# atomicarchitects/equiformer

Hardware: AMD Instinct MI355X
Metric: molecules/sec (train step) QM9 L_max=2, 6 blocks (higher is better)
Workload: dtype f32; 1 GPU; QM9 graph_attention_transformer_nonlinear_l2 train step (radius graph + fwd + L1 + bwd + AdamW), 128 molecules/GPU x 18 atoms, r=5.0, num_basis=128, alpha_drop=0.2; global_batch=128, nodes_per_gpu=2304, edges_per_gpu=25354, parallelism=dp1, matrix_mode=split, hip_graph=True, hip_graph_replays=452, hip_graph_eager_steps=3

## Files before the change

equiformer_amd/csrc/edge.hip:

```cpp
#include "common.h"
#include "prof.h"

namespace {

__global__ __launch_bounds__(256) void gather_add_kernel(const float* __restrict__ a, const float* __restrict__ b,
                                                         const int* __restrict__ src, const int* __restrict__ dst,
                                                         float* __restrict__ msg, long total4, int D4) {
  const long idx = (long)blockIdx.x * blockDim.x + threadIdx.x;
  if (idx >= total4) return;
  const long e = idx / D4;
  const int c = (int)(idx - e * D4);
  float4 v = reinterpret_cast<const float4*>(a)[(long)src[e] * D4 + c];
  if (b) {
    const float4 w = reinterpret_cast<const float4*>(b)[(long)dst[e] * D4 + c];
    v.x += w.x, v.y += w.y, v.z += w.z, v.w += w.w;
  }
  reinterpret_cast<float4*>(msg)[idx] = v;
}

__global__ __launch_bounds__(128) void segment_sum_kernel(const float* __restrict__ x, const int* __restrict__ ptr,
                                                          const int* __restrict__ perm, float* __restrict__ out, int D,
                                                          float scale, int accumulate) {
  const int n = blockIdx.x;
  const int beg = ptr[n], end = ptr[n + 1];
// ... 392 lines not shown
}

__global__ void attn_bwd_half_kernel(const float* __restrict__ alpha, const float* __restrict__ value,
                                     const int* __restrict__ row_ptr, const float* __restrict__ d_out,
                                     float* __restrict__ d_value, float* __restrict__ d_logit, const HeadTab T,
                                     float drop_p, unsigned long long seed0,
    const unsigned long long* __restrict__ seed_off) {
  const unsigned long long seed = seed0 + (seed_off ? *seed_off : 0ull);
  const int n = blockIdx.x;
  const int h = threadIdx.x >> 6, lane = threadIdx.x & 63;
  const int half = lane >> 5, gl = lane & 31;
  const int beg = row_ptr[n], end = row_ptr[n + 1];
  const int H = T.H, D4 = T.D >> 2;
  const int col4 = (gl < T.G) ? head_col(T, h, gl) >> 2 : -1;
  const float4 z4 = make_float4(0.f, 0.f, 0.f, 0.f);
  const float4 go = (col4 >= 0) ? reinterpret_cast<const float4*>(d_out)[(long)n * D4 + col4] : z4;
  float s_acc = 0.f;
  for (int e0 = beg; e0 < end; e0 += 4) {
    const int ea = e0 + half, eb = e0 + 2 + half;
    const bool va = ea < end, vb = eb < end;
    const float aa = va ? alpha[(long)ea * H + h] : 0.f, ab = vb ? alpha[(long)eb * H + h] : 0.f;
    const float4 xa = (va && col4 >= 0) ? reinterpret_cast<const float4*>(value)[(long)ea * D4 + col4] : z4;
    const float4 xb = (vb && col4 >= 0) ? reinterpret_cast<const float4*>(value)[(long)eb * D4 + col4] : z4;
    const float keepa = keep_scale(seed, (unsigned long long)ea * H + h, drop_p);
    const float keepb = keep_scale(seed, (unsigned long long)eb * H + h, drop_p);
    float pa = xa.x * go.x + xa.y * go.y + xa.z * go.z + xa.w * go.w;
    float pb = xb.x * go.x + xb.y * go.y + xb.z * go.z + xb.w * go.w;
    if (va && col4 >= 0) {
      const float k = aa * keepa;
      reinterpret_cast<float4*>(d_value)[(long)ea * D4 + col4] = make_float4(k * go.x, k * go.y, k * go.z, k * go.w);
    }
    if (vb && col4 >= 0) {
      const float k = ab * keepb;
      reinterpret_cast<float4*>(d_value)[(long)eb * D4 + col4] = make_float4(k * go.x, k * go.y, k * go.z, k * go.w);
    }
#pragma unroll
    for (int o = 16; o > 0; o >>= 1) pa += __shfl_xor(pa, o), pb += __shfl_xor(pb, o);
    const float da = pa * keepa, db = pb * keepb;
    float contrib = aa * da + ab * db;
    contrib += __shfl_xor(contrib, 32);
    s_acc += contrib;
    if (gl == 0) {
      if (va) d_logit[(long)ea * H + h] = da;
      if (vb) d_logit[(long)eb * H + h] = db;
    }
  }
  __threadfence_block();
  for (int e = beg + lane; e < end; e += 64) {
    const float da = d_logit[(long)e * H + h];
    d_logit[(long)e * H + h] = alpha[(long)e * H + h] * (da - s_acc);
  }
}

__global__ void attn_bwd_kernel(const float* __restrict__ alpha, const float* __restrict__ value,
                                const int* __restrict__ row_ptr, const float* __restrict__ d_out,
                                float* __restrict__ d_value, float* __restrict__ d_logit, const HeadTab T, float drop_p,
                                unsigned long long seed0,
    const unsigned long long* __restrict__ seed_off) {
  const unsigned long long seed = seed0 + (seed_off ? *seed_off : 0ull);
  const int n = blockIdx.x;
  const int h = threadIdx.x >> 6, lane = threadIdx.x & 63;
  const int beg = row_ptr[n], end = row_ptr[n + 1];
  const int H = T.H, D4 = T.D >> 2;
  int col4[MAX_SLOTS];
  float4 go[MAX_SLOTS];
#pragma unroll
  for (int s = 0; s < MAX_SLOTS; ++s) {
    const int g = lane + 64 * s;
    col4[s] = (g < T.G) ? head_col(T, h, g) >> 2 : -1;
    go[s] = (col4[s] >= 0) ? reinterpret_cast<const float4*>(d_out)[(long)n * D4 + col4[s]]
                           : make_float4(0.f, 0.f, 0.f, 0.f);
  }
  float s_acc = 0.f;
  for (int e = beg; e < end; ++e) {
    const float a = alpha[(long)e * H + h];
    const float keep = keep_scale(seed, (unsigned long long)e * H + h, drop_p);
    const float ak = a * keep;
    float part = 0.f;
#pragma unroll
    for (int s = 0; s < MAX_SLOTS; ++s)
      if (col4[s] >= 0) {
        const float4 v = reinterpret_cast<const float4*>(value)[(long)e * D4 + col4[s]];
        part += v.x * go[s].x + v.y * go[s].y + v.z * go[s].z + v.w * go[s].w;
        float4 dv;
        dv.x = ak * go[s].x, dv.y = ak * go[s].y, dv.z = ak * go[s].z, dv.w = ak * go[s].w;
        reinterpret_cast<float4*>(d_value)[(long)e * D4 + col4[s]] = dv;
      }
    const float da = wave_sum(part) * keep;
    s_acc = fmaf(a, da, s_acc);
    if (lane == 0) d_logit[(long)e * H + h] = da;
  }
  __threadfence_block();
  for (int e = beg + lane; e < end; e += 64) {
    const float da = d_logit[(long)e * H + h];
    d_logit[(long)e * H + h] = alpha[(long)e * H + h] * (da - s_acc);
  }
}

HeadTab make_headtab(const eqf_irreps& ir, int H, int* err) {
  HeadTab T{};
  *err = 0;
  T.nseg = ir.nseg;
  T.H = H;
  int off = 0, g = 0;
  for (int s = 0; s < ir.nseg; ++s) {
    T.off[s] = off;
// ... 156 lines not shown
  if (N <= 0) return 0;
  const int pid = eqf_prof_begin("attn_fwd", (hipStream_t)stream, 0.0, 0.0);
  if (T.G <= 32)
    hipLaunchKernelGGL(attn_fwd_half_kernel, dim3(N), dim3(64 * H), 0, (hipStream_t)stream, logit, value, row_ptr, alpha,
                       out, T, drop_p, seed, seed_off);
  else
    hipLaunchKernelGGL(attn_fwd_kernel, dim3(N), dim3(64 * H), 0, (hipStream_t)stream, logit, value, row_ptr, alpha, out,
                       T, drop_p, seed, seed_off);
  eqf_prof_end(pid, (hipStream_t)stream);
  EQF_CHECK_LAUNCH();
  return 0;
}

int eqf_attn_aggregate_fwd(const float* logit, const float* value, const int* row_ptr, float* alpha, float* out, int N,
                           int H, const eqf_irreps* irreps, float drop_p, unsigned long long seed, void* stream) {
  return attn_aggregate_fwd_impl(logit, value, row_ptr, alpha, out, N, H, irreps, drop_p, seed, nullptr, stream);
}
int eqf_attn_aggregate_fwd_dseed(const float* logit, const float* value, const int* row_ptr, float* alpha, float* out, int N,
                                 int H, const eqf_irreps* irreps, float drop_p, unsigned long long seed,
                                 const unsigned long long* seed_offset, void* stream) {
  return attn_aggregate_fwd_impl(logit, value, row_ptr, alpha, out, N, H, irreps, drop_p, seed, seed_offset, stream);
}

static int attn_aggregate_bwd_impl(const float* alpha, const float* value, const int* row_ptr, const float* d_out,
                                   float* d_value, float* d_logit, int N, int H, const eqf_irreps* irreps, float drop_p,
                                   unsigned long long seed, const unsigned long long* seed_off, void* stream) {
  if (!alpha || !value || !row_ptr || !d_out || !d_value || !d_logit || !irreps || H < 1) return EQF_E_BADARG;
  int err;
  const HeadTab T = make_headtab(*irreps, H, &err);
  if (err) return err;
  if (N <= 0) return 0;
  const int pid = eqf_prof_begin("attn_bwd", (hipStream_t)stream, 0.0, 0.0);
  if (T.G <= 32)
    hipLaunchKernelGGL(attn_bwd_half_kernel, dim3(N), dim3(64 * H), 0, (hipStream_t)stream, alpha, value, row_ptr, d_out,
                       d_value, d_logit, T, drop_p, seed, seed_off);
  else
    hipLaunchKernelGGL(attn_bwd_kernel, dim3(N), dim3(64 * H), 0, (hipStream_t)stream, alpha, value, row_ptr, d_out,
                       d_value, d_logit, T, drop_p, seed, seed_off);
  eqf_prof_end(pid, (hipStream_t)stream);
  EQF_CHECK_LAUNCH();
  return 0;
}
int eqf_attn_aggregate_bwd(const float* alpha, const float* value, const int* row_ptr, const float* d_out,
                           float* d_value, float* d_logit, int N, int H, const eqf_irreps* irreps, float drop_p,
                           unsigned long long seed, void* stream) {
  return attn_aggregate_bwd_impl(alpha, value, row_ptr, d_out, d_value, d_logit, N, H, irreps, drop_p, seed, nullptr, stream);
}
int eqf_attn_aggregate_bwd_dseed(const float* alpha, const float* value, const int* row_ptr, const float* d_out,
                                 float* d_value, float* d_logit, int N, int H, const eqf_irreps* irreps, float drop_p,
                                 unsigned long long seed, const unsigned long long* seed_offset, void* stream) {
  return attn_aggregate_bwd_impl(alpha, value, row_ptr, d_out, d_value, d_logit, N, H, irreps, drop_p, seed, seed_offset, stream);
}

}
```

equiformer_amd/lib.py:

```python
import ctypes
import os

_HERE = os.path.dirname(os.path.abspath(__file__))
LIB_PATH = os.path.join(_HERE, "libequiformer_hip.so")
if os.environ.get("EQF_LIB_VARIANT"):
    LIB_PATH = os.path.join(_HERE, "libequiformer_hip_%s.so" % os.environ["EQF_LIB_VARIANT"])

EQF_MAX_SEG = 8
EQF_MAX_PATHS = 72

c_fp = ctypes.c_void_p
c_int = ctypes.c_int


class EqfIrreps(ctypes.Structure):
    _fields_ = [("nseg", c_int), ("l", c_int * EQF_MAX_SEG), ("mul", c_int * EQF_MAX_SEG), ("odd", c_int * EQF_MAX_SEG)]


class EqfRows(ctypes.Structure):
    _fields_ = [("d", c_int), ("ld", c_int), ("inner", c_int)]


class EqfGemmDesc(ctypes.Structure):
    _fields_ = [("A", c_fp), ("B", c_fp), ("C", c_fp), ("bias", c_fp), ("ra", EqfRows), ("rc", EqfRows),
# ... 52 lines not shown
    "eqf_dtp_coupling_bwd": [c_fp, c_fp, _P_PATHS, c_fp, c_int, c_fp],
    "eqf_dtp_linear_fwd": [c_fp, c_fp, c_fp, _P_PATHS, _PP, c_fp, c_fp, _P_IRR, c_int, c_fp],
    "eqf_dtp_linear_wgrad": [c_fp, c_fp, c_fp, _P_PATHS, c_fp, _P_IRR, _PP, c_int, c_fp],
    "eqf_sfc_fwd": [c_fp, c_fp, c_fp, _P_PATHS, _PP, c_fp, c_fp, c_fp, c_fp, _P_IRR, c_fp, c_int, c_int, c_fp],
    "eqf_sfc_bwd_data": [c_fp, c_fp, c_fp, _P_PATHS, _PP, c_fp, c_fp, _P_IRR, c_fp, c_int, c_fp, c_fp, c_fp, c_int, c_fp],
    "eqf_sfc_bwd_weight": [c_fp, c_fp, c_fp, _P_PATHS, c_fp, _P_IRR, c_fp, c_int, _PP, c_fp, c_int, c_fp],
    "eqf_sfcx_packed_numel": [_P_PATHS, _P_IRR, c_int, c_int],
    "eqf_sfcx_supported": [_P_PATHS, _P_IRR, c_int, c_int],
    "eqf_sfcx_fwd_gated": [c_fp, ctypes.POINTER(EqfGateIn), c_fp, c_fp, _P_PATHS, c_fp, c_fp, c_fp, _P_IRR, c_int, c_int, c_fp],
    "eqf_sfcx_bwd_data_gated": [c_fp, ctypes.POINTER(EqfGateIn), c_fp, c_fp, _P_PATHS, c_fp, c_fp, _P_IRR, c_fp, c_fp, c_fp,
                                c_int, c_int, c_fp],
    "eqf_sfcx_bwd_weight_gated": [c_fp, ctypes.POINTER(EqfGateIn), c_fp, c_fp, _P_PATHS, c_fp, _P_IRR, _PP, c_int, c_int,
                                  c_fp],
    "eqf_sfcx_bwd_weight_bias": [c_fp, c_fp, c_fp, _P_PATHS, c_fp, _P_IRR, c_fp, c_int, _PP, c_fp, c_fp, c_fp, c_int, c_int, c_fp],
    "eqf_sfcx_bwd_weight_gated_bias": [c_fp, ctypes.POINTER(EqfGateIn), c_fp, c_fp, _P_PATHS, c_fp, _P_IRR, _PP, c_fp, c_int,
                                       c_int, c_fp],
    "eqf_sfcx_pack": [_PP, c_fp, _P_PATHS, _P_IRR, c_int, c_int, c_fp, c_fp],
    "eqf_sfcx_fwd": [c_fp, c_fp, c_fp, _P_PATHS, c_fp, c_fp, c_fp, c_fp, _P_IRR, c_fp, c_int, c_int, c_int, c_fp],
    "eqf_sfcx_bwd_data": [c_fp, c_fp, c_fp, _P_PATHS, c_fp, c_fp, _P_IRR, c_fp, c_int, c_fp, c_fp, c_fp, c_int, c_int, c_fp],
    "eqf_sfcx_bwd_weight": [c_fp, c_fp, c_fp, _P_PATHS, c_fp, _P_IRR, c_fp, c_int, _PP, c_fp, c_int, c_int, c_fp],
    "eqf_layernorm_fwd": [c_fp, c_fp, c_fp, c_fp, c_fp, c_fp, c_int, _P_IRR, _f, c_fp],
    "eqf_layernorm_bwd": [c_fp, c_fp, c_fp, c_fp, c_fp, c_fp, c_fp, c_fp, c_int, _P_IRR, c_fp],
    "eqf_add_layernorm_fwd": [c_fp, c_fp, c_fp, c_fp, c_fp, c_fp, c_fp, c_fp, c_int, _P_IRR, _f, c_fp],
    "eqf_add_layernorm_bwd": [c_fp, c_fp, c_fp, c_fp, c_fp, c_fp, c_fp, c_fp, c_fp, c_int, _P_IRR, c_fp],
    "eqf_gate_fwd": [c_fp, c_fp, c_int, c_int, _P_IRR, _f, _f, c_fp],
    "eqf_gate_bwd": [c_fp, c_fp, c_fp, c_int, c_int, _P_IRR, _f, _f, c_fp],
    "eqf_silu_fwd": [c_fp, c_fp, _long, _f, c_fp],
    "eqf_silu_bwd": [c_fp, c_fp, c_fp, _long, _f, c_fp],
    "eqf_lnsilu_fwd": [c_fp, c_fp, c_fp, c_fp, c_int, c_int, _f, c_fp],
    "eqf_lnsilu_bwd": [c_fp, c_fp, c_fp, c_fp, c_fp, c_fp, c_fp, c_int, c_int, _f, c_fp],
    "eqf_lnsilu_group_fwd": [c_fp, c_fp, c_fp, c_fp, c_int, c_int, c_int, _f, c_fp],
    "eqf_lnsilu_group_bwd": [c_fp, c_fp, c_fp, c_fp, c_fp, c_fp, c_fp, c_int, c_int, c_int, _f, c_fp],
    "eqf_fold_weight_fwd": [c_fp, c_fp, c_fp, c_fp, c_fp, c_int, c_fp],
    "eqf_fold_weight_bwd": [c_fp, c_fp, c_fp, c_fp, c_fp, c_fp, c_fp, c_int, c_fp],
    "eqf_embed_fwd": [c_fp, c_fp, c_fp, c_fp, c_int, c_int, c_int, c_fp],
    "eqf_embed_bwd": [c_fp, c_fp, c_fp, c_fp, c_int, c_int, c_int, c_fp],
    "eqf_gather_add_fwd": [c_fp, c_fp, c_fp, c_fp, c_fp, c_int, c_int, c_fp],
    "eqf_segment_sum": [c_fp, c_fp, c_fp, c_fp, c_int, c_int, _f, c_int, c_fp],
    "eqf_segment_bcast": [c_fp, c_fp, c_fp, c_int, c_int, _f, c_fp],
    "eqf_kv_split": [c_fp, c_fp, c_fp, c_int, c_int, c_fp, c_fp],
    "eqf_kv_merge": [c_fp, c_fp, c_fp, c_int, c_int, c_fp, c_fp],
    "eqf_dp_logits_fwd": [c_fp, c_fp, c_fp, c_fp, c_int, c_int, c_fp, c_fp],
    "eqf_dp_logits_bwd": [c_fp, c_fp, c_fp, c_fp, c_fp, c_fp, c_int, c_int, c_fp, c_fp],
    "eqf_vec_sh": [c_fp, c_fp, c_int, c_int, _f, c_fp, c_fp],
    "eqf_segment_scale": [c_fp, c_fp, c_fp, c_fp, c_int, c_int, c_fp],
    "eqf_dtp_fwd": [c_fp, c_fp, c_fp, _P_PATHS, c_fp, c_int, c_fp],
    "eqf_dtp_bwd": [c_fp, c_fp, c_fp, _P_PATHS, c_fp, c_fp, c_fp, c_fp, c_int, c_fp],
    "eqf_alpha_fwd": [c_fp, c_fp, c_fp, c_int, c_int, c_int, _f, c_fp],
    "eqf_alpha_bwd": [c_fp, c_fp, c_fp, c_fp, c_fp, c_int, c_int, c_int, _f, c_fp],
    "eqf_attn_aggregate_fwd": [c_fp, c_fp, c_fp, c_fp, c_fp, c_int, c_int, _P_IRR, _f, _u64, c_fp],
    "eqf_attn_aggregate_bwd": [c_fp, c_fp, c_fp, c_fp, c_fp, c_fp, c_int, c_int, _P_IRR, _f, _u64, c_fp],
    "eqf_attn_aggregate_fwd_dseed": [c_fp, c_fp, c_fp, c_fp, c_fp, c_int, c_int, _P_IRR, _f, _u64, c_fp, c_fp],
    "eqf_attn_aggregate_bwd_dseed": [c_fp, c_fp, c_fp, c_fp, c_fp, c_fp, c_int, c_int, _P_IRR, _f, _u64, c_fp, c_fp],
    "eqf_silu_bwd2": [c_fp, c_fp, c_fp, c_fp, c_fp, _long, _f, c_fp],
    "eqf_gate_bwd2": [c_fp, c_fp, c_fp, c_fp, c_fp, c_int, c_int, _P_IRR, _f, _f, c_fp],
    "eqf_lnsilu_bwd2": [c_fp, c_fp, c_fp, c_fp, c_fp, c_fp, c_fp, c_fp, c_fp, c_int, c_int, _f, c_fp],
    "eqf_lnsilu_group_bwd2": [c_fp, c_fp, c_fp, c_fp, c_fp, c_fp, c_fp, c_fp, c_fp, c_int, c_int, c_int, _f, c_fp],
    "eqf_layernorm_bwd2": [c_fp, c_fp, c_fp, c_fp, c_fp, c_fp, c_fp, c_int, _P_IRR, _f, c_fp],
    "eqf_alpha_bwd2": [c_fp, c_fp, c_fp, c_fp, c_fp, c_fp, c_fp, c_int, c_int, c_int, _f, c_fp],
    "eqf_attn_aggregate_bwd2": [c_fp, c_fp, c_fp, c_fp, c_fp, c_fp, c_fp, c_fp, c_fp, c_int, c_int, _P_IRR, _f, _u64,
                                c_fp],
    "eqf_rbf_expnorm_bwd2": [c_fp, c_fp, c_fp, c_int, c_int, c_fp, c_fp, _f, _f, c_fp, c_fp, c_fp],
    "eqf_rbf_gaussian_bwd2": [c_fp, c_fp, c_fp, c_int, c_int, c_fp, c_fp, c_fp, c_fp, _f, c_fp, c_fp, c_fp, c_fp, c_fp,
                              c_fp, c_fp],
    "eqf_rbf_bessel_bwd2": [c_fp, c_fp, c_fp, c_int, c_int, c_fp, _f, c_fp, c_fp, c_fp, c_fp],
    "eqf_edge_geom_bwd2": [c_fp, c_fp, c_fp, c_fp, c_int, c_int, c_fp, c_fp, c_fp, c_fp],
    "eqf_prof_enable": [ctypes.c_char_p],
    "eqf_prof_report": [ctypes.c_char_p, c_int],
}

RESTYPES = {"eqf_sfcx_packed_numel": ctypes.c_long}

_lib = None


class HipLibraryError(RuntimeError):
    pass


def load():
    global _lib
    if _lib is not None:
        return _lib
    if not os.path.exists(LIB_PATH):
        raise HipLibraryError(
            "libequiformer_hip.so not found at %s -- build it with `python -m equiformer_amd.build` "
            "(there is no CPU fallback for the hot path)" % LIB_PATH)
    lib = ctypes.CDLL(LIB_PATH)
    lib.eqf_version.restype = ctypes.c_char_p
    lib.eqf_version.argtypes = []
    for name, argtypes in SIGNATURES.items():
        fn = getattr(lib, name)
        fn.restype = RESTYPES.get(name, c_int)
        fn.argtypes = argtypes
    _check_build(lib)
    _lib = lib
    return lib


def _check_build(lib):
    csrc = os.path.join(_HERE, "csrc")
    if not os.path.isdir(csrc):
        return
    ver = lib.eqf_version().decode()
    built = ver.split("src=")[-1] if "src=" in ver else "unknown"
    from . import build as _build
# ... 58 lines not shown
```

equiformer_amd/nets/layers.py:

```python
import math
import os

import torch
from torch import nn

from .. import ops, so3
from ..irreps import Irrep, Irreps
from ..layout import DtpTable, RowLayout

_RESCALE = True
_USE_BIAS = True


def _simplified_sorted(irreps):
    irreps = Irreps(irreps)
    s, _ = irreps.sort_even_first()
    return s.simplify()


class _TensorProductWeights(nn.Module):

    def __init__(self, weight_numel, internal):
        super().__init__()
        self.weight_numel = weight_numel
# ... 411 lines not shown

        irreps_attn_heads = _simplified_sorted(self.irreps_head * num_heads)
        mul_alpha = sum(m for m, ir in irreps_attn_heads if ir.l == 0 and ir.p == 1)
        self.mul_alpha_head = mul_alpha // num_heads
        irreps_alpha = Irreps("{}x0e".format(mul_alpha))

        if nonlinear_message:
            self.sep_act = SeparableFCTP(self.irreps_pre_attn, self.irreps_edge_attr, self.irreps_pre_attn, fc_neurons,
                                         use_activation=True, norm_layer=None, internal_weights=False)
            self.sep_alpha = LinearRS(self.sep_act.dtp.table.irreps_out, irreps_alpha)
            self.sep_value = SeparableFCTP(self.irreps_pre_attn, self.irreps_edge_attr, irreps_attn_heads,
                                           fc_neurons=None, use_activation=False, norm_layer=None,
                                           internal_weights=True)
            self.alpha_fused_spec = (ops.DtpLinearSpec(self.sep_act.dtp.table, self.sep_alpha.layout_out)
                                     if self.sep_act.dtp.table.fusable and not self.sep_alpha.layout_out.has_odd else None)
            self.act_sfc_spec = ops.SfcSpec(self.sep_act.dtp.table, self.sep_act.lin.layout_out, n2=mul_alpha)
        else:
            irreps_attn_all = _simplified_sorted(irreps_alpha + irreps_attn_heads)
            self.sep = SeparableFCTP(self.irreps_pre_attn, self.irreps_edge_attr, irreps_attn_all, fc_neurons,
                                     use_activation=False, norm_layer=None, internal_weights=False)
            n0 = sum(m for m, ir in irreps_attn_all if ir.l == 0)
            hw = n0 // num_heads
            mah = self.mul_alpha_head
            self.register_buffer("_idx_alpha", torch.tensor([h * hw + k for h in range(num_heads) for k in range(mah)],
                                                            dtype=torch.long), persistent=False)
            self.register_buffer("_idx_value", torch.tensor([h * hw + mah + k for h in range(num_heads)
                                                             for k in range(hw - mah)], dtype=torch.long),
                                 persistent=False)
            self.lin_sfc_spec = ops.SfcSpec(self.sep.dtp.table, RowLayout(irreps_attn_heads), n2=mul_alpha)
            if not self.lin_sfc_spec.supported:
                raise NotImplementedError("linear-message attention needs the fused SeparableFCTP kernels "
                                          "(channel counts in multiples of 32)")
        self.heads_layout = RowLayout(irreps_attn_heads)

        self.alpha_dot = nn.Parameter(torch.randn(1, num_heads, self.mul_alpha_head))
        stdv = math.sqrt(6.0 / (self.alpha_dot.size(-2) + self.alpha_dot.size(-1)))
        self.alpha_dot.data.uniform_(-stdv, stdv)
        self.alpha_drop = float(alpha_drop)
        self.alpha_dropout = nn.Dropout(alpha_drop) if alpha_drop != 0.0 else None
        self.proj = LinearRS(irreps_attn_heads, self.irreps_node_output)
        self.proj_drop = None
        self.use_fused = True

    def forward(self, node_input, node_attr=None, edge_src=None, edge_dst=None, edge_attr=None, edge_scalars=None,
                batch=None, ectx=None, **kwargs):
        g = ectx.graph
        ms, md = ops.irreps_linear_pair(node_input, self.merge_src.tp.weight, self.merge_src._bias(), self.merge_src.spec,
                                        self.merge_dst.tp.weight, self.merge_dst._bias(), self.merge_dst.spec)
        message = ops.gather_add(ms, md, g)
        if not self.nonlinear_message:
            value, alpha = self._linear_message(message, ectx)
        else:
            value, alpha = self._nonlinear_message(message, ectx)
        logit = ops.alpha_logits(alpha, self.alpha_dot, self.num_heads, self.mul_alpha_head,
                                 so3.C_SMOOTH_LEAKY_RELU_02)
        drop_p, seed = 0.0, 0
        if self.training and self.alpha_drop > 0.0:
            drop_p = self.alpha_drop
            seed = int(torch.randint(0, 2 ** 62, (1,)).item())
        attn = ops.attn_aggregate(logit, value, g, self.num_heads, self.heads_layout, drop_p, seed)
        return self.proj(attn)

    def radial_module(self):
        return self.sep_act.dtp_rad if self.nonlinear_message else self.sep.dtp_rad

    def _nonlinear_message(self, message, ectx):
        sa = self.sep_act
        table = sa.dtp.table
        M = ectx.coupling(table)
        weight = ectx.radial(sa.dtp_rad)
        if self.use_fused is True and self.act_sfc_spec.supported:
            value, alpha = ops.sep_fctp(message, M, weight, sa.flat_weight(), sa.lin._bias(), self.act_sfc_spec,
                                        weight2=self.sep_alpha.tp.weight, bias2=self.sep_alpha._bias())
        elif self.use_fused and sa.fused_spec is not None:
            value = ops.dtp_linear(message, M, weight, sa.lin.tp.weight, sa.lin._bias(), sa.fused_spec)
            alpha = ops.dtp_linear(message, M, weight, self.sep_alpha.tp.weight, self.sep_alpha._bias(),
                                   self.alpha_fused_spec)
        else:
            mid = ops.dtp(message, M, weight, table)
            alpha = self.sep_alpha(mid)
            value = sa.lin(mid)
        sv = self.sep_value
        gt = sa.gate
        if (self.use_fused is True and isinstance(gt, Gate) and sv.gate is None
                and ops.sep_fctp_gated_ok(sv.sfc_spec, value.shape[1], gt.S, gt.gated_layout, E=value.shape[0])):
            w2 = ectx.radial(sv.dtp_rad) if sv.dtp_rad is not None else None
            value = ops.sep_fctp_gated(value, ectx.coupling(sv.dtp.table), w2, sv.flat_weight(), sv.lin._bias(), sv.sfc_spec,
                                       (gt.S, gt.gated_layout, so3.C_SILU, so3.C_SIGMOID))
        else:
            value = sv(gt(value), ectx, use_fused=self.use_fused)
        return value, alpha

    def _linear_message(self, message, ectx):
        sep = self.sep
        table = sep.dtp.table
        M = ectx.coupling(table)
        weight = ectx.radial(sep.dtp_rad)
        W = sep.lin.tp.weight
        (l, _, K0, _, N0, off0) = sep.lin.spec.pairs[0]
        assert l == 0 and off0 == 0
        W0 = W[:K0 * N0].view(K0, N0)
        w_main = torch.cat([W0.index_select(1, self._idx_value).reshape(-1), W[K0 * N0:]])
        w_alpha = W0.index_select(1, self._idx_alpha).reshape(-1)
        b = sep.lin._bias()
        return ops.sep_fctp(message, M, weight, w_main, b.index_select(0, self._idx_value), self.lin_sfc_spec,
                            weight2=w_alpha, bias2=b.index_select(0, self._idx_alpha))


class DotProductAttention(nn.Module):

    def __init__(self, irreps_node_input, irreps_node_attr, irreps_edge_attr, irreps_node_output, fc_neurons,
                 irreps_head, num_heads, irreps_pre_attn=None, rescale_degree=False, alpha_drop=0.1, proj_drop=0.1):
        super().__init__()
# ... 213 lines not shown
```

equiformer_amd/ops.py:

```python
import contextlib
import ctypes
import os
import weakref

import torch
from torch.autograd import Function
from torch.autograd.function import once_differentiable

from . import lib
from .lib import EqfGemmDesc, EqfRows, call


class HipOnlyError(RuntimeError):
    pass


_dummy = {}


class _Flag:
    on = False


_input_grads_only = _Flag()
# ... 2272 lines not shown
    def backward(ctx, dout):
        alpha, value, logit = ctx.saved_tensors
        graph, H, layout, drop_p, seed = ctx.args
        if torch.is_grad_enabled():
            if ctx.seed_off is not None:
                raise NotImplementedError("second-order backward of a captured step with attention dropout")
            dlogit, dvalue = _AttnAggregateBwd.apply(logit, value, dout, alpha, graph, H, layout, drop_p, seed)
            return dlogit, dvalue, None, None, None, None, None
        dout = _c(dout)
        _chk(dout)
        dvalue = torch.empty_like(value)
        dlogit = torch.empty_like(alpha)
        if ctx.seed_off is None:
            call("eqf_attn_aggregate_bwd", _p(alpha), _p(value), _p(graph.row_ptr), _p(dout), _p(dvalue), _p(dlogit),
                 graph.N, H, layout.c_ref, drop_p, seed, _stream())
        else:
            call("eqf_attn_aggregate_bwd_dseed", _p(alpha), _p(value), _p(graph.row_ptr), _p(dout), _p(dvalue), _p(dlogit),
                 graph.N, H, layout.c_ref, drop_p, seed, _p(ctx.seed_off), _stream())
        return dlogit, dvalue, None, None, None, None, None


class _AttnAggregateBwd(Function):

    @staticmethod
    def forward(ctx, logit, value, dout, alpha, graph, H, layout, drop_p, seed):
        dout = _c(dout)
        _chk(dout)
        dvalue = torch.empty_like(value)
        dlogit = torch.empty_like(alpha)
        call("eqf_attn_aggregate_bwd", _p(alpha), _p(value), _p(graph.row_ptr), _p(dout), _p(dvalue), _p(dlogit),
             graph.N, H, layout.c_ref, drop_p, seed, _stream())
        ctx.save_for_backward(alpha, value, dout)
        ctx.args = (graph, H, layout, drop_p, seed)
        return dlogit, dvalue

    @staticmethod
    @once_differentiable
    def backward(ctx, cl, cv):
        alpha, value, dout = ctx.saved_tensors
        graph, H, layout, drop_p, seed = ctx.args
        cl = _c(cl) if cl is not None else None
        cv = _c(cv) if cv is not None else None
        _chk(cl, cv)
        g_logit, g_value, g_dout = torch.empty_like(alpha), torch.empty_like(value), torch.empty_like(dout)
        call("eqf_attn_aggregate_bwd2", _p(alpha), _p(value), _p(graph.row_ptr), _p(dout), _p(cv), _p(cl), _p(g_logit),
             _p(g_value), _p(g_dout), graph.N, H, layout.c_ref, drop_p, seed, _stream())
        return g_logit, g_value, g_dout, None, None, None, None, None, None


def attn_aggregate(logit, value, graph, H, layout, drop_p=0.0, seed=0):
    return _AttnAggregate.apply(logit, value, graph, H, layout, float(drop_p), int(seed))


class _KvSplit(Function):

    @staticmethod
    def forward(ctx, kv, H, layout):
        kv = _c(kv)
        _chk(kv)
        E = kv.shape[0]
        assert kv.shape[1] == 2 * layout.dim
        k = torch.empty((E, layout.dim), device=kv.device, dtype=torch.float32)
        v = torch.empty_like(k)
        call("eqf_kv_split", _p(kv), _p(k), _p(v), E, H, layout.c_ref, _stream())
        ctx.args = (H, layout)
        return k, v

    @staticmethod
    def backward(ctx, dk, dv):
        H, layout = ctx.args
        return _KvMerge.apply(dk, dv, H, layout), None, None


class _KvMerge(Function):
    @staticmethod
    def forward(ctx, k, v, H, layout):
        ref = k if k is not None else v
        k = _c(k) if k is not None else None
        v = _c(v) if v is not None else None
        _chk(k, v)
        kv = torch.empty((ref.shape[0], 2 * layout.dim), device=ref.device, dtype=torch.float32)
        call("eqf_kv_merge", _p(k), _p(v), _p(kv), ref.shape[0], H, layout.c_ref, _stream())
        ctx.args = (H, layout)
        return kv

    @staticmethod
    def backward(ctx, dkv):
        H, layout = ctx.args
        k, v = _KvSplit.apply(dkv, H, layout)
        return k, v, None, None


def kv_split(kv, H, layout):
    return _KvSplit.apply(kv, H, layout)


def _dp_logits_fwd(q, k, graph, H, layout):
    logit = torch.empty((k.shape[0], H), device=k.device, dtype=torch.float32)
    call("eqf_dp_logits_fwd", _p(q), _p(k), _p(graph.dst), _p(logit), k.shape[0], H, layout.c_ref, _stream())
    return logit


def _dp_logits_bwd(q, k, dlogit, graph, H, layout, want_q, want_k):
    dq = torch.empty((graph.N, layout.dim), device=dlogit.device, dtype=torch.float32) if want_q else None
    dk = torch.empty((dlogit.shape[0], layout.dim), device=dlogit.device, dtype=torch.float32) if want_k else None
    call("eqf_dp_logits_bwd", _p(q) if want_k else None, _p(k) if want_q else None, _p(dlogit), _p(graph.row_ptr), _p(dq),
# ... 59 lines not shown
```

include/equiformer_hip.h:

```cpp
#ifndef EQUIFORMER_HIP_H
#define EQUIFORMER_HIP_H

#ifdef __cplusplus
extern "C" {
#endif

#define EQF_MAX_SEG 8
#define EQF_MAX_PATHS 72

#define EQF_E_BADARG (-1)
#define EQF_E_UNSUPPORTED (-2)

typedef struct eqf_irreps {
  int nseg;
  int l[EQF_MAX_SEG];
  int mul[EQF_MAX_SEG];
  int odd[EQF_MAX_SEG];
} eqf_irreps;

typedef struct eqf_dtp_paths {
  int npaths;
  int sh_dim;
  int in_dim;
  int out_dim;
// ... 169 lines not shown

int eqf_lnsilu_group_fwd(const float* x, const float* gamma, const float* beta, float* y, int rows, int C, int groups,
                         float eps, void* stream);
int eqf_lnsilu_group_bwd(const float* x, const float* gamma, const float* beta, const float* dy, float* dx,
                         float* d_gamma, float* d_beta, int rows, int C, int groups, float eps, void* stream);

int eqf_fold_weight_fwd(const float* W, const float* w, const int* row_start, const int* w_of_row, float* out, int rows,
                        void* stream);
int eqf_fold_weight_bwd(const float* W, const float* w, const int* row_start, const int* w_of_row, const float* g,
                        float* dW, float* dw, int rows, void* stream);

int eqf_embed_fwd(const int* type, const float* W, const float* b, float* y, int rows, int C, int D,
                  void* stream);
int eqf_embed_bwd(const int* type, const float* dy, float* dW, float* db, int rows, int C, int D,
                  void* stream);


int eqf_gather_add_fwd(const float* a, const float* b, const int* src, const int* dst, float* msg,
                       int E, int D, void* stream);

int eqf_segment_sum(const float* x, const int* ptr, const int* perm, float* out, int nseg, int D,
                    float scale, int accumulate, void* stream);
int eqf_segment_bcast(const float* x, const int* seg_of, float* out, int rows, int D, float scale,
                      void* stream);

int eqf_segment_scale(const float* x, const float* s, const int* seg_of, float* out, int rows, int D,
                      void* stream);

int eqf_dtp_fwd(const float* x, const float* coupling, const float* w, const eqf_dtp_paths* paths,
                float* out, int E, void* stream);
int eqf_dtp_bwd(const float* x, const float* coupling, const float* w, const eqf_dtp_paths* paths,
                const float* d_out, float* dx, float* dw, float* d_coupling, int E, void* stream);

int eqf_alpha_fwd(const float* a, const float* alpha_dot, float* logit, int E, int H, int Kh, float c,
                  void* stream);
int eqf_alpha_bwd(const float* a, const float* alpha_dot, const float* d_logit, float* da,
                  float* d_alpha_dot, int E, int H, int Kh, float c, void* stream);

int eqf_attn_aggregate_fwd(const float* logit, const float* value, const int* row_ptr, float* alpha,
                           float* out, int N, int H, const eqf_irreps* irreps, float drop_p,
                           unsigned long long seed, void* stream);
int eqf_attn_aggregate_bwd(const float* alpha, const float* value, const int* row_ptr,
                           const float* d_out, float* d_value, float* d_logit, int N, int H,
                           const eqf_irreps* irreps, float drop_p, unsigned long long seed,
                           void* stream);

int eqf_attn_aggregate_fwd_dseed(const float* logit, const float* value, const int* row_ptr, float* alpha,
                                 float* out, int N, int H, const eqf_irreps* irreps, float drop_p,
                                 unsigned long long seed, const unsigned long long* seed_offset, void* stream);
int eqf_attn_aggregate_bwd_dseed(const float* alpha, const float* value, const int* row_ptr,
                                 const float* d_out, float* d_value, float* d_logit, int N, int H,
                                 const eqf_irreps* irreps, float drop_p, unsigned long long seed,
                                 const unsigned long long* seed_offset, void* stream);

int eqf_kv_split(const float* kv, float* k, float* v, int E, int H, const eqf_irreps* irreps, void* stream);
int eqf_kv_merge(const float* k, const float* v, float* kv, int E, int H, const eqf_irreps* irreps, void* stream);
int eqf_dp_logits_fwd(const float* q, const float* k, const int* dst, float* logit, int E, int H,
                      const eqf_irreps* irreps, void* stream);
int eqf_dp_logits_bwd(const float* q, const float* k, const float* d_logit, const int* row_ptr, float* dq, float* dk,
                      int N, int H, const eqf_irreps* irreps, void* stream);

int eqf_silu_bwd2(const float* x, const float* dy, const float* c, float* g_x, float* g_dy, long n, float c0,
                  void* stream);
int eqf_gate_bwd2(const float* in, const float* d_out, const float* c, float* g_in, float* g_dout, int rows, int S,
                  const eqf_irreps* gated, float c_silu, float c_sig, void* stream);
int eqf_lnsilu_bwd2(const float* x, const float* gamma, const float* beta, const float* dy, const float* c,
                    float* g_x, float* g_gamma, float* g_beta, float* g_dy, int rows, int C, float eps, void* stream);
int eqf_lnsilu_group_bwd2(const float* x, const float* gamma, const float* beta, const float* dy, const float* c,
                          float* g_x, float* g_gamma, float* g_beta, float* g_dy, int rows, int C, int groups, float eps,
                          void* stream);
int eqf_layernorm_bwd2(const float* x, const float* weight, const float* dy, const float* c, float* g_x,
                       float* g_weight, float* g_dy, int rows, const eqf_irreps* irreps, float eps, void* stream);
int eqf_alpha_bwd2(const float* a, const float* alpha_dot, const float* d_logit, const float* ca, float* g_a,
                   float* g_alpha_dot, float* g_dlogit, int E, int H, int Kh, float c, void* stream);
int eqf_attn_aggregate_bwd2(const float* alpha, const float* value, const int* row_ptr, const float* d_out,
                            const float* c_value, const float* c_logit, float* g_logit, float* g_value,
                            float* g_dout, int N, int H, const eqf_irreps* irreps, float drop_p,
                            unsigned long long seed, void* stream);
int eqf_rbf_expnorm_bwd2(const float* len, const float* d_out, const float* c_len, int E, int R, const float* means,
                         const float* betas, float alpha, float cutoff, float* g_len, float* g_dout, void* stream);
int eqf_rbf_gaussian_bwd2(const float* len, const float* d_out, const float* c_len, int E, int R, const float* mean,
                          const float* std, const float* weight, const float* bias, float cutoff, float* g_len,
                          float* g_dout, float* g_mean, float* g_std, float* g_weight, float* g_bias, void* stream);
int eqf_rbf_bessel_bwd2(const float* len, const float* d_out, const float* c_len, int E, int R, const float* freq,
                        float cutoff, float* g_len, float* g_dout, float* g_freq, void* stream);
int eqf_edge_geom_bwd2(const float* vec, const float* d_sh, const float* d_len, const float* c_vec, int E, int lmax,
                       float* g_vec, float* g_dsh, float* g_dlen, void* stream);


int eqf_prof_enable(const char* filter);
int eqf_prof_report(char* buf, int buflen);

int eqf_sumsq(const float* g, long n, float* out, void* stream);
int eqf_adamw_step(float* p, const float* g, float* m, float* v, const float* wd, float* ema, const float* sumsq,
                   long n, float lr, float beta1, float beta2, float eps, int step, float max_norm, float ema_decay,
                   void* stream);
int eqf_adamw_step_dev(float* p, const float* g, float* m, float* v, const float* wd, float* ema, const float* sumsq,
                       long n, const float* hyper, float beta1, float beta2, float eps, float max_norm,
                       float ema_decay, void* stream);

#ifdef __cplusplus
}
#endif
#endif
```

Baseline: 14240 molecules/s.

## Fuse alpha logit computation into attention aggregate forward and backward kernels

Adds fused kernels that compute the smooth-leaky-ReLU alpha logits (dot with alpha_dot per head) inside the softmax/aggregate kernel, and in backward fuse the aggregate backward with the logit backward, emitting per-node partial alpha_dot gradients reduced by a colsum. This removes separate alpha_logits and alpha_bwd launches and the materialized logit/d_logit round trips through memory. In exchange, logits are recomputed per pass (up to three times for high-degree nodes), some work uses double accumulation, and the fused path only applies when Kh is 32 and the per-head group fits in 32 lanes.

```diff
diff --git a/equiformer_amd/csrc/edge.hip b/equiformer_amd/csrc/edge.hip
--- a/equiformer_amd/csrc/edge.hip
+++ b/equiformer_amd/csrc/edge.hip
@@ -468,6 +468,193 @@
   }
 }
 
+constexpr int LG_PF = 8;
+
+__device__ __forceinline__ float half_logit(float av, float ad, float c) {
+#pragma clang fp contract(off)
+  const float s = sigmoidf_(av);
+  float v = ad * (c * fmaf(0.4f * av, fmaf(s, 2.f, -1.f), 0.6f * av));
+#pragma unroll
+  for (int o = 16; o > 0; o >>= 1) v += __shfl_xor(v, o);
+  return v;
+}
+
+__device__ __forceinline__ float chunk_logits(const float* __restrict__ a, int e0, int cnt, int HK, int col, float ad, float c,
+                                              int lane) {
+  const int half = lane >> 5;
+  float lg = -INFINITY;
+  for (int s = 0; s < cnt; s += 2 * LG_PF) {
+    float x[LG_PF];
+#pragma unroll
+    for (int u = 0; u < LG_PF; ++u) {
+      const int i = s + 2 * u + half;
+      x[u] = i < cnt ? a[(long)(e0 + i) * HK + col] : 0.f;
+    }
+#pragma unroll
+    for (int u = 0; u < LG_PF; ++u) {
+      const float v = half_logit(x[u], ad, c);
+      const float v0 = __shfl(v, 0), v1 = __shfl(v, 32);
+      const int i = s + 2 * u;
+      if (lane == i && i < cnt) lg = v0;
+      if (lane == i + 1 && i + 1 < cnt) lg = v1;
+    }
+  }
+  return lg;
+}
+
+__global__ void attn_logits_fwd_half_kernel(const float* __restrict__ a, const float* __restrict__ adot, float c,
+                                            const float* __restrict__ value, const int* __restrict__ row_ptr,
+                                            float* __restrict__ alpha, float* __restrict__ out, const HeadTab T, float drop_p,
+                                            unsigned long long seed0, const unsigned long long* __restrict__ seed_off) {
+  const unsigned long long seed = seed0 + (seed_off ? *seed_off : 0ull);
+  const int n = blockIdx.x;
+  const int h = threadIdx.x >> 6, lane = threadIdx.x & 63;
+  const int half = lane >> 5, gl = lane & 31;
+  const int beg = row_ptr[n], end = row_ptr[n + 1];
+  const int H = T.H, D4 = T.D >> 2, HK = H * 32;
+  const int deg = end - beg;
+  const int col4 = (gl < T.G) ? head_col(T, h, gl) >> 2 : -1;
+  const int col = h * 32 + gl;
+  const float4 z4 = make_float4(0.f, 0.f, 0.f, 0.f);
+  const float4* const V = reinterpret_cast<const float4*>(value);
+  float4 xa = (beg + half < end && col4 >= 0) ? V[(long)(beg + half) * D4 + col4] : z4;
+  float4 xb = (beg + 2 + half < end && col4 >= 0) ? V[(long)(beg + 2 + half) * D4 + col4] : z4;
+  const float ad = adot[col];
+  const float lg = chunk_logits(a, beg, min(deg, 64), HK, col, ad, c, lane);
+  float mx = lg;
+  for (int cb = 64; cb < deg; cb += 64)
+    mx = fmaxf(mx, chunk_logits(a, beg + cb, min(deg - cb, 64), HK, col, ad, c, lane));
+  mx = wave_max(mx);
+  float sm = lane < deg ? __expf(lg - mx) : 0.f;
+  for (int cb = 64; cb < deg; cb += 64) {
+    const float l2 = chunk_logits(a, beg + cb, min(deg - cb, 64), HK, col, ad, c, lane);
+    if (cb + lane < deg) sm += __expf(l2 - mx);
+  }
+  sm = wave_sum(sm);
+  const float inv = 1.f / (sm + 1e-16f);
+  float4 acc = make_float4(0.f, 0.f, 0.f, 0.f);
+  for (int e0 = beg; e0 < end; e0 += 4) {
+    const int ea = e0 + half, eb = e0 + 2 + half;
+    const bool va = ea < end, vb = eb < end;
+    const float4 xan = (ea + 4 < end && col4 >= 0) ? V[(long)(ea + 4) * D4 + col4] : z4;
+    const float4 xbn = (eb + 4 < end && col4 >= 0) ? V[(long)(eb + 4) * D4 + col4] : z4;
+    const int ia = ea - beg, ib = eb - beg;
+    float la = __shfl(lg, ia & 63), lb = __shfl(lg, ib & 63);
+    if (e0 - beg >= 64) {
+      la = half_logit(va ? a[(long)ea * HK + col] : 0.f, ad, c);
+      lb = half_logit(vb ? a[(long)eb * HK + col] : 0.f, ad, c);
+    }
+    const float aa = va ? __expf(la - mx) * inv : 0.f, ab = vb ? __expf(lb - mx) * inv : 0.f;
+    if (gl == 0) {
+      if (va) alpha[(long)ea * H + h] = aa;
+      if (vb) alpha[(long)eb * H + h] = ab;
+    }
+    const float ka = aa * keep_scale(seed, (unsigned long long)ea * H + h, drop_p);
+    const float kb = ab * keep_scale(seed, (unsigned long long)eb * H + h, drop_p);
+    acc.x = fmaf(ka, xa.x, acc.x), acc.y = fmaf(ka, xa.y, acc.y), acc.z = fmaf(ka, xa.z, acc.z), acc.w = fmaf(ka, xa.w, acc.w);
+    acc.x = fmaf(kb, xb.x, acc.x), acc.y = fmaf(kb, xb.y, acc.y), acc.z = fmaf(kb, xb.z, acc.z), acc.w = fmaf(kb, xb.w, acc.w);
+    xa = xan, xb = xbn;
+  }
+  acc.x += __shfl_xor(acc.x, 32), acc.y += __shfl_xor(acc.y, 32);
+  acc.z += __shfl_xor(acc.z, 32), acc.w += __shfl_xor(acc.w, 32);
+  if (half == 0 && col4 >= 0) reinterpret_cast<float4*>(out)[(long)n * D4 + col4] = acc;
+}
+
+__global__ void attn_logits_bwd_half_kernel(const float* __restrict__ a, const float* __restrict__ adot, float c,
+                                            const float* __restrict__ alpha, const float* __restrict__ value,
+                                            const int* __restrict__ row_ptr, const float* __restrict__ d_out,
+                                            float* __restrict__ d_value, float* __restrict__ da_out,
+                                            float* __restrict__ dd_rows, const HeadTab T, float drop_p,
+                                            unsigned long long seed0, const unsigned long long* __restrict__ seed_off) {
+  const unsigned long long seed = seed0 + (seed_off ? *seed_off : 0ull);
+  const int n = blockIdx.x;
+  const int h = threadIdx.x >> 6, lane = threadIdx.x & 63;
+  const int half = lane >> 5, gl = lane & 31;
+  const int beg = row_ptr[n], end = row_ptr[n + 1];
+  const int H = T.H, D4 = T.D >> 2, HK = H * 32;
+  const int deg = end - beg;
+  const int col = h * 32 + gl;
+  if (deg <= 0) {
+    if (half == 0) dd_rows[(long)n * HK + col] = 0.f;
+    return;
+  }
+  const int col4 = (gl < T.G) ? head_col(T, h, gl) >> 2 : -1;
+  const float4 z4 = make_float4(0.f, 0.f, 0.f, 0.f);
+  const float4 go = (col4 >= 0) ? reinterpret_cast<const float4*>(d_out)[(long)n * D4 + col4] : z4;
+  float ap[LG_PF];
+#pragma unroll
+  for (int u = 0; u < LG_PF; ++u) ap[u] = (2 * u + half < deg) ? a[(long)(beg + 2 * u + half) * HK + col] : 0.f;
+  const float al0 = lane < deg ? alpha[(long)(beg + lane) * H + h] : 0.f;
+  const float ad = adot[col];
+  float dal = 0.f;
+  float s_acc = 0.f;
+  for (int e0 = beg; e0 < end; e0 += 4) {
+    const int ea = e0 + half, eb = e0 + 2 + half;
+    const bool va = ea < end, vb = eb < end;
+    const float aa = va ? alpha[(long)ea * H + h] : 0.f, ab = vb ? alpha[(long)eb * H + h] : 0.f;
+    const float4 xa = (va && col4 >= 0) ? reinterpret_cast<const float4*>(value)[(long)ea * D4 + col4] : z4;
+    const float4 xb = (vb && col4 >= 0) ? reinterpret_cast<const float4*>(value)[(long)eb * D4 + col4] : z4;
+    const float keepa = keep_scale(seed, (unsigned long long)ea * H + h, drop_p);
+    const float keepb = keep_scale(seed, (unsigned long long)eb * H + h, drop_p);
+    float pa = xa.x * go.x + xa.y * go.y + xa.z * go.z + xa.w * go.w;
+    float pb = xb.x * go.x + xb.y * go.y + xb.z * go.z + xb.w * go.w;
+    if (va && col4 >= 0) {
+      const float k = aa * keepa;
+      reinterpret_cast<float4*>(d_value)[(long)ea * D4 + col4] = make_float4(k * go.x, k * go.y, k * go.z, k * go.w);
+    }
+    if (vb && col4 >= 0) {
+      const float k = ab * keepb;
+      reinterpret_cast<float4*>(d_value)[(long)eb * D4 + col4] = make_float4(k * go.x, k * go.y, k * go.z, k * go.w);
+    }
+#pragma unroll
+    for (int o = 16; o > 0; o >>= 1) pa += __shfl_xor(pa, o), pb += __shfl_xor(pb, o);
+    const float da = pa * keepa, db = pb * keepb;
+    float contrib = aa * da + ab * db;
+    contrib += __shfl_xor(contrib, 32);
+    s_acc += contrib;
+    const int i0 = e0 - beg;
+    if (i0 < 64) {
+      const float d0 = __shfl(da, 0), d1 = __shfl(da, 32), d2 = __shfl(db, 0), d3 = __shfl(db, 32);
+      const int r = lane - i0;
+      if (r >= 0 && r < 4) dal = r == 0 ? d0 : r == 1 ? d1 : r == 2 ? d2 : d3;
+    } else if (gl == 0) {
+      if (va) da_out[(long)ea * HK + h * 32] = da;
+      if (vb) da_out[(long)eb * HK + h * 32] = db;
+    }
+  }
+  if (deg > 64) __threadfence_block();
+  double acc = 0.0;
+  for (int cb = 0; cb < deg; cb += 64) {
+    const int cnt = min(deg - cb, 64);
+    float g = 0.f;
+    if (cb == 0) {
+      g = (al0 * (dal - s_acc)) * c;
+    } else if (lane < cnt) {
+      const long e = beg + cb + lane;
+      g = (alpha[e * H + h] * (da_out[e * HK + h * 32] - s_acc)) * c;
+    }
+    for (int s = 0; s < cnt; s += 2 * LG_PF) {
+      float x[LG_PF];
+#pragma unroll
+      for (int u = 0; u < LG_PF; ++u) {
+        const int i = s + 2 * u + half;
+        x[u] = (cb == 0 && s == 0) ? ap[u] : (i < cnt ? a[(long)(beg + cb + i) * HK + col] : 0.f);
+      }
+#pragma unroll
+      for (int u = 0; u < LG_PF; ++u) {
+        const int i = s + 2 * u + half;
+        const float ge = __shfl(g, i & 63);
+        if (i < cnt) {
+          da_out[(long)(beg + cb + i) * HK + col] = ge * ad * dslrelu(x[u]);
+          acc += (double)ge * (double)slrelu(x[u]);
+        }
+      }
+    }
+  }
+  acc += __shfl_xor(acc, 32);
+  if (half == 0) dd_rows[(long)n * HK + col] = (float)acc;
+}
+
 __global__ void attn_bwd_kernel(const float* __restrict__ alpha, const float* __restrict__ value,
                                 const int* __restrict__ row_ptr, const float* __restrict__ d_out,
                                 float* __restrict__ d_value, float* __restrict__ d_logit, const HeadTab T, float drop_p,
@@ -730,4 +917,84 @@
   return attn_aggregate_bwd_impl(alpha, value, row_ptr, d_out, d_value, d_logit, N, H, irreps, drop_p, seed, seed_offset, stream);
 }
 
-}
+static int attn_logits_tab(int H, int Kh, const eqf_irreps* irreps, HeadTab* T) {
+  if (!irreps || H < 1) return EQF_E_BADARG;
+  int err;
+  *T = make_headtab(*irreps, H, &err);
+  if (err) return err;
+  if (Kh != 32 || T->G > 32) return EQF_E_UNSUPPORTED;
+  return 0;
+}
+
+int eqf_attn_logits_supported(int H, int Kh, const eqf_irreps* irreps) {
+  HeadTab T;
+  const int rc = attn_logits_tab(H, Kh, irreps, &T);
+  return rc == 0 ? 1 : (rc == EQF_E_UNSUPPORTED ? 0 : rc);
+}
+
+static int attn_logits_aggregate_fwd_impl(const float* a, const float* alpha_dot, float c, const float* value,
+                                          const int* row_ptr, float* alpha, float* out, int N, int H, int Kh,
+                                          const eqf_irreps* irreps, float drop_p, unsigned long long seed,
+                                          const unsigned long long* seed_off, void* stream) {
+  if (!a || !alpha_dot || !value || !row_ptr || !alpha || !out) return EQF_E_BADARG;
+  HeadTab T;
+  const int rc = attn_logits_tab(H, Kh, irreps, &T);
+  if (rc) return rc;
+  if (N <= 0) return 0;
+  const int pid = eqf_prof_begin("attn_fwd", (hipStream_t)stream, 0.0, 0.0);
+  hipLaunchKernelGGL(attn_logits_fwd_half_kernel, dim3(N), dim3(64 * H), 0, (hipStream_t)stream, a, alpha_dot, c, value,
+                     row_ptr, alpha, out, T, drop_p, seed, seed_off);
+  eqf_prof_end(pid, (hipStream_t)stream);
+  EQF_CHECK_LAUNCH();
+  return 0;
+}
+
+int eqf_attn_logits_aggregate_fwd(const float* a, const float* alpha_dot, float c, const float* value, const int* row_ptr,
+                                  float* alpha, float* out, int N, int H, int Kh, const eqf_irreps* irreps, float drop_p,
+                                  unsigned long long seed, void* stream) {
+  return attn_logits_aggregate_fwd_impl(a, alpha_dot, c, value, row_ptr, alpha, out, N, H, Kh, irreps, drop_p, seed, nullptr,
+                                        stream);
+}
+int eqf_attn_logits_aggregate_fwd_dseed(const float* a, const float* alpha_dot, float c, const float* value,
+                                        const int* row_ptr, float* alpha, float* out, int N, int H, int Kh,
+                                        const eqf_irreps* irreps, float drop_p, unsigned long long seed,
+                                        const unsigned long long* seed_offset, void* stream) {
+  return attn_logits_aggregate_fwd_impl(a, alpha_dot, c, value, row_ptr, alpha, out, N, H, Kh, irreps, drop_p, seed,
+                                        seed_offset, stream);
+}
+
+static int attn_logits_aggregate_bwd_impl(const float* a, const float* alpha_dot, float c, const float* alpha,
+                                          const float* value, const int* row_ptr, const float* d_out, float* d_value,
+                                          float* da, float* d_alpha_dot_rows, int N, int H, int Kh, const eqf_irreps* irreps,
+                                          float drop_p, unsigned long long seed, const unsigned long long* seed_off,
+                                          void* stream) {
+  if (!a || !alpha_dot || !alpha || !value || !row_ptr || !d_out || !d_value || !da || !d_alpha_dot_rows) return EQF_E_BADARG;
+  HeadTab T;
+  const int rc = attn_logits_tab(H, Kh, irreps, &T);
+  if (rc) return rc;
+  if (N <= 0) return 0;
+  const int pid = eqf_prof_begin("attn_bwd", (hipStream_t)stream, 0.0, 0.0);
+  hipLaunchKernelGGL(attn_logits_bwd_half_kernel, dim3(N), dim3(64 * H), 0, (hipStream_t)stream, a, alpha_dot, c, alpha,
+                     value, row_ptr, d_out, d_value, da, d_alpha_dot_rows, T, drop_p, seed, seed_off);
+  eqf_prof_end(pid, (hipStream_t)stream);
+  EQF_CHECK_LAUNCH();
+  return 0;
+}
+
+int eqf_attn_logits_aggregate_bwd(const float* a, const float* alpha_dot, float c, const float* alpha, const float* value,
+                                  const int* row_ptr, const float* d_out, float* d_value, float* da, float* d_alpha_dot_rows,
+                                  int N, int H, int Kh, const eqf_irreps* irreps, float drop_p, unsigned long long seed,
+                                  void* stream) {
+  return attn_logits_aggregate_bwd_impl(a, alpha_dot, c, alpha, value, row_ptr, d_out, d_value, da, d_alpha_dot_rows, N, H, Kh,
+                                        irreps, drop_p, seed, nullptr, stream);
+}
+int eqf_attn_logits_aggregate_bwd_dseed(const float* a, const float* alpha_dot, float c, const float* alpha,
+                                        const float* value, const int* row_ptr, const float* d_out, float* d_value,
+                                        float* da, float* d_alpha_dot_rows, int N, int H, int Kh, const eqf_irreps* irreps,
+                                        float drop_p, unsigned long long seed, const unsigned long long* seed_offset,
+                                        void* stream) {
+  return attn_logits_aggregate_bwd_impl(a, alpha_dot, c, alpha, value, row_ptr, d_out, d_value, da, d_alpha_dot_rows, N, H, Kh,
+                                        irreps, drop_p, seed, seed_offset, stream);
+}
+
+}
diff --git a/equiformer_amd/lib.py b/equiformer_amd/lib.py
--- a/equiformer_amd/lib.py
+++ b/equiformer_amd/lib.py
@@ -128,6 +128,14 @@
     "eqf_attn_aggregate_bwd": [c_fp, c_fp, c_fp, c_fp, c_fp, c_fp, c_int, c_int, _P_IRR, _f, _u64, c_fp],
     "eqf_attn_aggregate_fwd_dseed": [c_fp, c_fp, c_fp, c_fp, c_fp, c_int, c_int, _P_IRR, _f, _u64, c_fp, c_fp],
     "eqf_attn_aggregate_bwd_dseed": [c_fp, c_fp, c_fp, c_fp, c_fp, c_fp, c_int, c_int, _P_IRR, _f, _u64, c_fp, c_fp],
+    "eqf_attn_logits_supported": [c_int, c_int, _P_IRR],
+    "eqf_attn_logits_aggregate_fwd": [c_fp, c_fp, _f, c_fp, c_fp, c_fp, c_fp, c_int, c_int, c_int, _P_IRR, _f, _u64, c_fp],
+    "eqf_attn_logits_aggregate_bwd": [c_fp, c_fp, _f, c_fp, c_fp, c_fp, c_fp, c_fp, c_fp, c_fp, c_int, c_int, c_int, _P_IRR,
+                                      _f, _u64, c_fp],
+    "eqf_attn_logits_aggregate_fwd_dseed": [c_fp, c_fp, _f, c_fp, c_fp, c_fp, c_fp, c_int, c_int, c_int, _P_IRR, _f, _u64,
+                                            c_fp, c_fp],
+    "eqf_attn_logits_aggregate_bwd_dseed": [c_fp, c_fp, _f, c_fp, c_fp, c_fp, c_fp, c_fp, c_fp, c_fp, c_int, c_int, c_int,
+                                            _P_IRR, _f, _u64, c_fp, c_fp],
     "eqf_silu_bwd2": [c_fp, c_fp, c_fp, c_fp, c_fp, _long, _f, c_fp],
     "eqf_gate_bwd2": [c_fp, c_fp, c_fp, c_fp, c_fp, c_int, c_int, _P_IRR, _f, _f, c_fp],
     "eqf_lnsilu_bwd2": [c_fp, c_fp, c_fp, c_fp, c_fp, c_fp, c_fp, c_fp, c_fp, c_int, c_int, _f, c_fp],
diff --git a/equiformer_amd/nets/layers.py b/equiformer_amd/nets/layers.py
--- a/equiformer_amd/nets/layers.py
+++ b/equiformer_amd/nets/layers.py
@@ -487,13 +487,12 @@
             value, alpha = self._linear_message(message, ectx)
         else:
             value, alpha = self._nonlinear_message(message, ectx)
-        logit = ops.alpha_logits(alpha, self.alpha_dot, self.num_heads, self.mul_alpha_head,
-                                 so3.C_SMOOTH_LEAKY_RELU_02)
         drop_p, seed = 0.0, 0
         if self.training and self.alpha_drop > 0.0:
             drop_p = self.alpha_drop
             seed = int(torch.randint(0, 2 ** 62, (1,)).item())
-        attn = ops.attn_aggregate(logit, value, g, self.num_heads, self.heads_layout, drop_p, seed)
+        attn = ops.attn_logits_aggregate(alpha, self.alpha_dot, value, g, self.num_heads, self.mul_alpha_head,
+                                         so3.C_SMOOTH_LEAKY_RELU_02, self.heads_layout, drop_p, seed)
         return self.proj(attn)
 
     def radial_module(self):
diff --git a/equiformer_amd/ops.py b/equiformer_amd/ops.py
--- a/equiformer_amd/ops.py
+++ b/equiformer_amd/ops.py
@@ -2348,6 +2348,75 @@
     return _AttnAggregate.apply(logit, value, graph, H, layout, float(drop_p), int(seed))
 
 
+class _AttnLogitsAggregate(Function):
+
+    @staticmethod
+    def forward(ctx, a, alpha_dot, value, graph, H, Kh, c, layout, drop_p, seed):
+        a, alpha_dot, value = _c(a), _c(alpha_dot), _c(value)
+        _chk(a, alpha_dot, value)
+        N = graph.N
+        alpha = torch.empty((a.shape[0], H), device=a.device, dtype=torch.float32)
+        out = torch.empty((N, layout.dim), device=value.device, dtype=torch.float32)
+        off = _seed_offset[0] if drop_p > 0.0 else None
+        if off is None:
+            call("eqf_attn_logits_aggregate_fwd", _p(a), _p(alpha_dot), c, _p(value), _p(graph.row_ptr), _p(alpha), _p(out),
+                 N, H, Kh, layout.c_ref, drop_p, seed, _stream())
+        else:
+            call("eqf_attn_logits_aggregate_fwd_dseed", _p(a), _p(alpha_dot), c, _p(value), _p(graph.row_ptr), _p(alpha),
+                 _p(out), N, H, Kh, layout.c_ref, drop_p, seed, _p(off), _stream())
+        ctx.save_for_backward(a, alpha_dot, value, alpha)
+        ctx.args = (graph, H, Kh, c, layout, drop_p, seed)
+        ctx.seed_off = off
+        return out
+
+    @staticmethod
+    def backward(ctx, dout):
+        a, alpha_dot, value, alpha = ctx.saved_tensors
+        graph, H, Kh, c, layout, drop_p, seed = ctx.args
+        if torch.is_grad_enabled():
+            if ctx.seed_off is not None:
+                raise NotImplementedError("second-order backward of a captured step with attention dropout")
+            logit = alpha_logits(a, alpha_dot, H, Kh, c)
+            dlogit, dvalue = _AttnAggregateBwd.apply(logit, value, dout, alpha, graph, H, layout, drop_p, seed)
+            da, dd = _AlphaLogitsBwd.apply(a, alpha_dot, dlogit, H, Kh, c)
+            return da, _guard(dd, dlogit, "alpha_dot gradient"), dvalue, None, None, None, None, None, None, None
+        dout = _c(dout)
+        _chk(dout)
+        dvalue = torch.empty_like(value)
+        da = torch.empty_like(a)
+        N, HK, st = graph.N, H * Kh, _stream()
+        dd_rows = torch.empty((N, HK), device=a.device, dtype=torch.float32)
+        if ctx.seed_off is None:
+            call("eqf_attn_logits_aggregate_bwd", _p(a), _p(alpha_dot), c, _p(alpha), _p(value), _p(graph.row_ptr), _p(dout),
+                 _p(dvalue), _p(da), _p(dd_rows), N, H, Kh, layout.c_ref, drop_p, seed, st)
+        else:
+            call("eqf_attn_logits_aggregate_bwd_dseed", _p(a), _p(alpha_dot), c, _p(alpha), _p(value), _p(graph.row_ptr),
+                 _p(dout), _p(dvalue), _p(da), _p(dd_rows), N, H, Kh, layout.c_ref, drop_p, seed, _p(ctx.seed_off), st)
+        dd = _zeros_like(alpha_dot)
+        call("eqf_colsum", _p(dd_rows), rows(1, HK, 0), N, HK, _p(dd), st)
+        return da, dd, dvalue, None, None, None, None, None, None, None
+
+
+_attn_fused_shapes = {}
+
+
+def _attn_fused_supported(H, Kh, layout):
+    key = (H, Kh, tuple(layout.segs))
+    ok = _attn_fused_shapes.get(key)
+    if ok is None:
+        rc = lib.load().eqf_attn_logits_supported(H, Kh, layout.c_ref)
+        if rc < 0:
+            raise lib.HipLibraryError("eqf_attn_logits_supported failed with code %d" % rc)
+        ok = _attn_fused_shapes[key] = bool(rc)
+    return ok
+
+
+def attn_logits_aggregate(a, alpha_dot, value, graph, H, Kh, c, layout, drop_p=0.0, seed=0):
+    if _attn_fused_supported(H, Kh, layout):
+        return _AttnLogitsAggregate.apply(a, alpha_dot, value, graph, H, Kh, float(c), layout, float(drop_p), int(seed))
+    return attn_aggregate(alpha_logits(a, alpha_dot, H, Kh, c), value, graph, H, layout, drop_p, seed)
+
+
 class _KvSplit(Function):
 
     @staticmethod
diff --git a/include/equiformer_hip.h b/include/equiformer_hip.h
--- a/include/equiformer_hip.h
+++ b/include/equiformer_hip.h
@@ -245,6 +245,24 @@
                                  const float* d_out, float* d_value, float* d_logit, int N, int H,
                                  const eqf_irreps* irreps, float drop_p, unsigned long long seed,
                                  const unsigned long long* seed_offset, void* stream);
+
+int eqf_attn_logits_supported(int H, int Kh, const eqf_irreps* irreps);
+int eqf_attn_logits_aggregate_fwd(const float* a, const float* alpha_dot, float c, const float* value,
+                                  const int* row_ptr, float* alpha, float* out, int N, int H, int Kh,
+                                  const eqf_irreps* irreps, float drop_p, unsigned long long seed, void* stream);
+int eqf_attn_logits_aggregate_bwd(const float* a, const float* alpha_dot, float c, const float* alpha,
+                                  const float* value, const int* row_ptr, const float* d_out, float* d_value,
+                                  float* da, float* d_alpha_dot_rows, int N, int H, int Kh, const eqf_irreps* irreps,
+                                  float drop_p, unsigned long long seed, void* stream);
+int eqf_attn_logits_aggregate_fwd_dseed(const float* a, const float* alpha_dot, float c, const float* value,
+                                        const int* row_ptr, float* alpha, float* out, int N, int H, int Kh,
+                                        const eqf_irreps* irreps, float drop_p, unsigned long long seed,
+                                        const unsigned long long* seed_offset, void* stream);
+int eqf_attn_logits_aggregate_bwd_dseed(const float* a, const float* alpha_dot, float c, const float* alpha,
+                                        const float* value, const int* row_ptr, const float* d_out, float* d_value,
+                                        float* da, float* d_alpha_dot_rows, int N, int H, int Kh, const eqf_irreps* irreps,
+                                        float drop_p, unsigned long long seed, const unsigned long long* seed_offset,
+                                        void* stream);
 
 int eqf_kv_split(const float* kv, float* k, float* v, int E, int H, const eqf_irreps* irreps, void* stream);
 int eqf_kv_merge(const float* k, const float* v, float* kv, int E, int H, const eqf_irreps* irreps, void* stream);
```

Result: no change. 14360 molecules/s, median of 6 (+0.9%).
